# SowpatiLab/ribbit

Hardware: AMD Instinct MI355X
Metric: Gbases/s scanned (m=2..100) (higher is better)
Workload: dtype u32 bit planes

## Files before the change

ribbit_amd/csrc/kernels.hip:

```cpp
#include <hip/hip_runtime.h>

#include <algorithm>
#include <climits>
#include <type_traits>

#include "kernels.h"

namespace rb {

__device__ __forceinline__ uint32_t funnel(uint32_t hi, uint32_t lo, uint32_t sh) {
    return __builtin_amdgcn_alignbit(hi, lo, sh);
}

template <unsigned TT>
__device__ __forceinline__ uint32_t bitop3(uint32_t a, uint32_t b, uint32_t c) {
    return __builtin_amdgcn_bitop3_b32(a, b, c, TT);
}

__global__ __launch_bounds__(256) void pack_kernel(const uint8_t *__restrict__ ascii, int64_t length,
                                                   uint32_t *__restrict__ hi, uint32_t *__restrict__ lo,
                                                   uint32_t *__restrict__ brk, int64_t total_words,
                                                   uint32_t *__restrict__ zero_words, int n_zero) {
    const int64_t t = (int64_t)blockIdx.x * blockDim.x + threadIdx.x;
    if (blockIdx.x == 0)
        for (int i = threadIdx.x; i < n_zero; i += 256) zero_words[i] = 0u;
    if (t >= total_words) return;
    const int64_t p0 = (t - LEAD_WORDS) * 32;
    uint32_t h = 0, l = 0, b = 0xffffffffu;
    if (p0 >= 0 && p0 < length) {
        uint32_t w[8];
        const int64_t left = length - p0;
        const uint8_t *src = ascii + p0;
        if (left >= 32 && (((uintptr_t)src) & 15) == 0) {
            const uint4 v0 = *reinterpret_cast<const uint4 *>(src);
            const uint4 v1 = *reinterpret_cast<const uint4 *>(src + 16);
            w[0] = v0.x; w[1] = v0.y; w[2] = v0.z; w[3] = v0.w;
            w[4] = v1.x; w[5] = v1.y; w[6] = v1.z; w[7] = v1.w;
        } else {
#pragma unroll
            for (int i = 0; i < 8; i++) {
                uint32_t x = 0;
#pragma unroll
                for (int k = 0; k < 4; k++) {
                    const int idx = 4 * i + k;
                    const uint32_t c = (idx < left) ? (uint32_t)src[idx] : (uint32_t)'N';
                    x |= c << (8 * k);
                }
                w[i] = x;
            }
        }
        b = 0;
#pragma unroll
        for (int i = 0; i < 8; i++) {
            const uint32_t x = w[i];
            const uint32_t b2 = (x >> 2) & 0x01010101u;
            const uint32_t lo1 = ((x >> 1) & 0x01010101u) ^ b2;
            const uint32_t both = lo1 & b2, either = lo1 | b2;
            uint32_t expect = (either << 1) + 0x61616161u;
            expect = (b2 << 2) + expect;
            expect = (both << 3) + expect;
            expect = (both << 2) + expect;
            expect = both + expect;
            const uint32_t diff = (x | 0x20202020u) ^ expect;
            const uint32_t nz = (((diff & 0x7f7f7f7fu) + 0x7f7f7f7fu) | diff) & 0x80808080u;
            const uint32_t bad = nz >> 7;
            const uint32_t ok = bad ^ 0x01010101u;
            const uint32_t weights = 0x08040201u;
            h |= __builtin_amdgcn_udot4(b2 & ok, weights, 0u, false) << (4 * i);
            l |= __builtin_amdgcn_udot4(lo1 & ok, weights, 0u, false) << (4 * i);
            b |= __builtin_amdgcn_udot4(bad, weights, 0u, false) << (4 * i);
        }
        if (left < 32) b |= 0xffffffffu << (uint32_t)left;
    }
    hi[t] = h; lo[t] = l; brk[t] = b;
}

void launch_pack(const uint8_t *dev_ascii, int64_t length, uint32_t *hi, uint32_t *lo, uint32_t *brk,
                 int64_t total_words, uint32_t *zero_words, int n_zero, hipStream_t stream) {
    const int threads = 256;
    const int64_t blocks = (total_words + threads - 1) / threads;
    hipLaunchKernelGGL(pack_kernel, dim3((unsigned)blocks), dim3(threads), 0, stream, dev_ascii, length, hi, lo, brk,
                       total_words, zero_words, n_zero);
}

constexpr int EV_STAGE = 256;

__device__ __forceinline__ int wave_inclusive_scan(int v) {
    v += __builtin_amdgcn_update_dpp(0, v, 0x111, 0xf, 0xf, true);
    v += __builtin_amdgcn_update_dpp(0, v, 0x112, 0xf, 0xf, true);
    v += __builtin_amdgcn_update_dpp(0, v, 0x114, 0xf, 0xf, true);
    v += __builtin_amdgcn_update_dpp(0, v, 0x118, 0xf, 0xf, true);
    v += __builtin_amdgcn_update_dpp(0, v, 0x142, 0xa, 0xf, false);
    v += __builtin_amdgcn_update_dpp(0, v, 0x143, 0xc, 0xf, false);
    return v;
}

struct EventSink {
    uint64_t *events;
    uint32_t *counters;
    uint32_t region_cap;
    uint32_t shard;
};

__device__ __forceinline__ void sink_flush(const EventSink &sk, volatile uint64_t *stage, int &staged, int lane) {
    if (staged == 0) return;
    uint32_t base = 0;
    if (lane == 0) base = atomicAdd(&sk.counters[sk.shard * EV_COUNTER_STRIDE], (uint32_t)staged);
    base = (uint32_t)__builtin_amdgcn_readfirstlane((int)base);
    uint64_t *dst = sk.events + (size_t)sk.shard * sk.region_cap;
    for (int i = lane; i < staged; i += 64) {
        const uint32_t idx = base + (uint32_t)i;
        if (idx < sk.region_cap) dst[idx] = stage[i];
    }
    __builtin_amdgcn_wave_barrier();
    staged = 0;
}

template <typename EndKind>
__device__ __forceinline__ void stage_events(const uint32_t (&S)[WORDS_PER_LANE], const uint32_t (&E)[WORDS_PER_LANE],
                                             uint32_t word0, uint32_t mlen, const EventSink &sink,
                                             volatile uint64_t *stage, int &staged, int lane, EndKind end_kind) {
    uint32_t Sv[WORDS_PER_LANE], Ev[WORDS_PER_LANE];
#pragma unroll
    for (int k = 0; k < WORDS_PER_LANE; k++) {
        Sv[k] = S[k]; Ev[k] = E[k];
        asm volatile("" : "+v"(Sv[k]), "+v"(Ev[k]));
    }
    int cnt = 0;
#pragma unroll
    for (int k = 0; k < WORDS_PER_LANE; k++) cnt += __popc(Sv[k]) + __popc(Ev[k]);
    const int incl = wave_inclusive_scan(cnt);
    const int total = __builtin_amdgcn_readlane(incl, 63);
    if (staged + total > EV_STAGE) sink_flush(sink, stage, staged, lane);
    const bool direct = total > EV_STAGE;
    uint32_t idx = (uint32_t)(incl - cnt);
    uint64_t *gdst = nullptr;
    if (direct) {
        uint32_t base = 0;
        if (lane == 0) base = atomicAdd(&sink.counters[sink.shard * EV_COUNTER_STRIDE], (uint32_t)total);
        idx += (uint32_t)__builtin_amdgcn_readfirstlane((int)base);
        gdst = sink.events + (size_t)sink.shard * sink.region_cap;
    } else {
        idx += (uint32_t)staged;
    }
#pragma unroll
    for (int k = 0; k < WORDS_PER_LANE; k++) {
        uint32_t both = Sv[k] | Ev[k];
        while (both) {
            const uint32_t b = (uint32_t)__builtin_ctz(both);
            both &= both - 1u;
            const uint32_t pos = ((word0 + (uint32_t)k) << 5) + b;
            const uint32_t kind = ((Sv[k] >> b) & 1u) ? (uint32_t)EV_START : end_kind(k, b, pos);
            const uint64_t e = ev_pack(pos, mlen, kind);
            if (direct) { if (idx < sink.region_cap) gdst[idx] = e; }
            else stage[idx] = e;
            idx++;
        }
    }
    if (!direct) staged += total;
    __builtin_amdgcn_wave_barrier();
}

constexpr int K = WORDS_PER_LANE;

#ifndef RB_COOP_MAX_LANES
#define RB_COOP_MAX_LANES 16
#endif
constexpr int COOP_SRC = 16;
struct CoopScratch { uint32_t w[COOP_SRC][20]; };

__device__ __forceinline__ void stage_events_coop(const uint32_t (&S)[WORDS_PER_LANE], const uint32_t (&E)[WORDS_PER_LANE], uint32_t word0, uint32_t mlen,
                                                  uint32_t brk_at, const uint32_t *s_brk, uint32_t length, CoopScratch &sc, const EventSink &sink,
                                                  volatile uint64_t *stage, int &staged, int lane) {
    uint32_t Sv[WORDS_PER_LANE], Ev[WORDS_PER_LANE];
#pragma unroll
    for (int k = 0; k < WORDS_PER_LANE; k++) {
        Sv[k] = S[k]; Ev[k] = E[k];
        asm volatile("" : "+v"(Sv[k]), "+v"(Ev[k]));
    }
    int cnt = 0;
#pragma unroll
    for (int k = 0; k < WORDS_PER_LANE; k++) cnt += __popc(Sv[k] | Ev[k]);
    const int incl = wave_inclusive_scan(cnt);
    const int total = __builtin_amdgcn_readlane(incl, 63);
    if (staged + total > EV_STAGE) sink_flush(sink, stage, staged, lane);
    const bool direct = total > EV_STAGE;
    uint32_t first = (uint32_t)(incl - cnt);
    uint64_t *gdst = nullptr;
    if (direct) {
        uint32_t base = 0;
        if (lane == 0) base = atomicAdd(&sink.counters[sink.shard * EV_COUNTER_STRIDE], (uint32_t)total);
        first += (uint32_t)__builtin_amdgcn_readfirstlane((int)base);
        gdst = sink.events + (size_t)sink.shard * sink.region_cap;
    } else {
        first += (uint32_t)staged;
    }
    unsigned long long todo = __ballot(cnt != 0);
    const int r = lane >> 2, j = lane & 3;
    do {
        const int rank = (int)__builtin_amdgcn_mbcnt_hi((uint32_t)(todo >> 32), __builtin_amdgcn_mbcnt_lo((uint32_t)todo, 0u));
        const bool mine = ((todo >> lane) & 1ull) != 0ull && rank < COOP_SRC;
        if (mine) {
            uint32_t *row = sc.w[rank];
#pragma unroll
            for (int k = 0; k < WORDS_PER_LANE; k++) { row[k] = Sv[k]; row[WORDS_PER_LANE + k] = Ev[k]; }
            row[16] = word0; row[17] = mlen; row[18] = brk_at; row[19] = first;
        }
        const unsigned long long handled = __ballot(mine);
        const int nsrc = __popcll(handled);
        todo &= ~handled;
        __builtin_amdgcn_wave_barrier();
        uint32_t s0 = 0, s1 = 0, e0 = 0, e1 = 0;
        if (r < nsrc) { s0 = sc.w[r][2 * j]; s1 = sc.w[r][2 * j + 1]; e0 = sc.w[r][WORDS_PER_LANE + 2 * j]; e1 = sc.w[r][WORDS_PER_LANE + 2 * j + 1]; }
        const int c = __popc(s0 | e0) + __popc(s1 | e1);
        const int q0 = __builtin_amdgcn_update_dpp(0, c, 0x00, 0xf, 0xf, true);
        const int q1 = __builtin_amdgcn_update_dpp(0, c, 0x55, 0xf, 0xf, true);
        const int q2 = __builtin_amdgcn_update_dpp(0, c, 0xaa, 0xf, 0xf, true);
        if (c != 0) {
            const uint32_t w0 = sc.w[r][16], ml = sc.w[r][17], bb = sc.w[r][18];
            uint32_t idx = sc.w[r][19] + (uint32_t)((j > 0 ? q0 : 0) + (j > 1 ? q1 : 0) + (j > 2 ? q2 : 0));
            auto expand = [&](uint32_t sw, uint32_t ew, uint32_t k) {
                uint32_t both = sw | ew;
                while (both) {
                    const uint32_t b = (uint32_t)__builtin_ctz(both);
                    both &= both - 1u;
                    const uint32_t pos = ((w0 + k) << 5) + b;
                    uint32_t kind = (uint32_t)EV_START;
                    if (!((sw >> b) & 1u))
                        kind = pos >= length ? (uint32_t)EV_END_EOS : (((s_brk[bb + k] >> b) & 1u) ? (uint32_t)EV_END_N : (uint32_t)EV_END_ZERO);
                    const uint64_t e = ev_pack(pos, ml, kind);
                    if (direct) { if (idx < sink.region_cap) gdst[idx] = e; }
                    else stage[idx] = e;
                    idx++;
                }
            };
            expand(s0, e0, 2u * (uint32_t)j);
            expand(s1, e1, 2u * (uint32_t)j + 1u);
        }
        __builtin_amdgcn_wave_barrier();
    } while (RB_COOP_MAX_LANES > COOP_SRC && todo != 0ull);
    if (!direct) staged += total;
}
__device__ __forceinline__ void group_filter(const uint32_t (&PASS)[K + 2], const uint32_t (&EVAL)[K + 2], int tj, uint32_t (&SV)[K + 1],
                                             uint32_t (&DR)[K]) {
    uint32_t J[K + 2], W[K + 2];
#pragma unroll
    for (int j = K + 1; j >= 1; j--) J[j] = PASS[j] | funnel(PASS[j], PASS[j - 1], 31);
    J[0] = PASS[0] | (PASS[0] << 1);
#pragma unroll
    for (int j = K + 1; j >= 1; j--) J[j] = J[j] | funnel(J[j], J[j - 1], 30);
    J[0] = J[0] | (J[0] << 2);
#pragma unroll
    for (int j = K + 1; j >= 1; j--) J[j] = J[j] | funnel(J[j], J[j - 1], 28);
    J[0] = J[0] | (J[0] << 4);
#pragma unroll
    for (int j = 0; j < K + 1; j++) J[j] = J[j] & funnel(J[j + 1], J[j], 1);
    J[K + 1] = J[K + 1] & (J[K + 1] >> 1);
#pragma unroll
    for (int j = 0; j < K + 1; j++) J[j] = J[j] & funnel(J[j + 1], J[j], 2);
    J[K + 1] = J[K + 1] & (J[K + 1] >> 2);
#pragma unroll
    for (int j = 0; j < K + 1; j++) J[j] = J[j] & funnel(J[j + 1], J[j], 4);
    J[K + 1] = J[K + 1] & (J[K + 1] >> 4);
#pragma unroll
    for (int j = 0; j < K + 2; j++) J[j] |= PASS[j];
#pragma unroll
    for (int j = 0; j < K + 2; j++) W[j] = J[j];
    {
        int span = 1;
#pragma unroll
        for (int step = 0; step < 4; step++) {
            const int sh = min(span, tj - span);
            if (sh > 0) {
#pragma unroll
                for (int j = 0; j < K + 1; j++) W[j] = W[j] & funnel(W[j + 1], W[j], (uint32_t)sh);
                W[K + 1] = W[K + 1] & (W[K + 1] >> sh);
                span += sh;
            }
        }
        span = 1;
#pragma unroll
        for (int step = 0; step < 4; step++) {
            const int sh = min(span, tj - span);
            if (sh > 0) {
#pragma unroll
                for (int j = K + 1; j >= 1; j--) W[j] = W[j] | funnel(W[j], W[j - 1], (uint32_t)(32 - sh));
                W[0] = W[0] | (W[0] << sh);
                span += sh;
            }
        }
    }
    auto special_ends = [&](int j) {
        const uint32_t jprev = j > 0 ? funnel(J[j], J[j - 1], 31) : (J[0] << 1);
        const uint32_t ev8 = j < K + 1 ? funnel(EVAL[j + 1], EVAL[j], 8) : (EVAL[K + 1] >> 8);
        const uint32_t g = ~J[j] & jprev & ~(EVAL[j] & ev8);
        return j == 0 ? 0u : (j == K + 1 ? (g & 0x0000ffffu) : g);
    };
    uint32_t special = 0;
#pragma unroll
    for (int j = 1; j < K + 2; j++) special |= special_ends(j);
    if (__ballot(special != 0) != 0ull) {
        uint32_t G[K + 2], JL[K + 2];
#pragma unroll
        for (int j = 0; j < K + 2; j++) { JL[j] = J[j]; G[j] = special_ends(j); }
#pragma unroll
        for (int j = 0; j < K + 1; j++) G[j] = funnel(G[j + 1], G[j], 1) & J[j];
        G[K + 1] = (G[K + 1] >> 1) & J[K + 1];
#pragma unroll
        for (int sh = 1; sh <= 8; sh <<= 1) {
#pragma unroll
            for (int j = 0; j < K + 1; j++) G[j] |= funnel(G[j + 1], G[j], (uint32_t)sh) & JL[j];
            G[K + 1] |= (G[K + 1] >> sh) & JL[K + 1];
#pragma unroll
            for (int j = 0; j < K + 1; j++) JL[j] = JL[j] & funnel(JL[j + 1], JL[j], (uint32_t)sh);
            JL[K + 1] = JL[K + 1] & (JL[K + 1] >> sh);
        }
#pragma unroll
        for (int j = 0; j < K + 1; j++) W[j] |= G[j];
    }
#pragma unroll
    for (int j = 0; j < K + 1; j++) SV[j] = W[j];
#pragma unroll
    for (int k = 0; k < K; k++) {
        const uint32_t jprev = funnel(J[k + 1], J[k], 31);
        const uint32_t svprev = funnel(W[k + 1], W[k], 31);
        DR[k] = ~J[k + 1] & jprev & ~svprev;
    }
}

constexpr int LDS_EXTRA = 40;

template <bool UNIFORM>
__device__ __forceinline__ uint32_t perfect_edges(const uint32_t (&Z)[K + 2], uint32_t t3, uint32_t t4, uint32_t t5,
                                                  uint32_t back, uint32_t (&SQ)[K], uint32_t (&EQ)[K]) {
    uint32_t D[K + 2];
#pragma unroll
    for (int j = 0; j < K + 1; j++) D[j] = Z[j] | funnel(Z[j + 1], Z[j], 1);
    D[K + 1] = Z[K + 1] | (Z[K + 1] >> 1);
#pragma unroll
    for (int j = 0; j < K + 1; j++) D[j] = D[j] | funnel(D[j + 1], D[j], 2);
    D[K + 1] = D[K + 1] | (D[K + 1] >> 2);
#pragma unroll
    for (int j = 0; j < K + 1; j++) D[j] = D[j] | funnel(D[j + 1], D[j], t3);
    D[K + 1] = D[K + 1] | (D[K + 1] >> t3);
#pragma unroll
    for (int j = 0; j < K + 1; j++) D[j] = D[j] | funnel(D[j + 1], D[j], t4);
    if (!UNIFORM || t5) {
        D[K + 1] = D[K + 1] | (D[K + 1] >> t4);
#pragma unroll
        for (int j = 0; j < K + 1; j++) D[j] = D[j] | funnel(D[j + 1], D[j], t5);
    }
    uint32_t any = 0;
#pragma unroll
    for (int k = 0; k < K; k++) {
        const int j = k + 1;
        const uint32_t prev_z = funnel(Z[j], Z[j - 1], 31);
        const uint32_t d_back = funnel(D[j], D[j - 1], back);
        SQ[k] = prev_z & ~D[j];
        EQ[k] = Z[j] & ~d_back;
        any = bitop3<0xFE>(SQ[k], EQ[k], any);
    }
    return any;
}

constexpr int CAND_CAP = 64;
#ifndef RB_CAND_DIRECT
#define RB_CAND_DIRECT 32
#endif
constexpr int CAND_DIRECT = RB_CAND_DIRECT;
struct CandQueue {
    uint32_t z[K + 2][CAND_CAP];
    uint32_t tag[CAND_CAP];
};

#ifndef RB_PERFECT_WAVES
#define RB_PERFECT_WAVES 4
#endif
__global__ __launch_bounds__(256) __attribute__((amdgpu_waves_per_eu(RB_PERFECT_WAVES, RB_PERFECT_WAVES))) void scan_perfect_kernel(DevicePlanes pl, PerfectLaunch pp, int motifs_per_block,
                                                           uint64_t *__restrict__ events,
                                                           uint32_t *__restrict__ counters) {
    __shared__ uint32_t s_hi[TILE_WORDS + LDS_EXTRA];
    __shared__ uint32_t s_lo[TILE_WORDS + LDS_EXTRA];
    __shared__ uint32_t s_brk[TILE_WORDS + 8];
    __shared__ uint64_t s_stage[4][EV_STAGE];
    __shared__ CandQueue s_cand[4];
    __shared__ CoopScratch s_coop[4];

    const int lane = threadIdx.x & 63;
    const int wave = __builtin_amdgcn_readfirstlane((int)(threadIdx.x >> 6));
    const int64_t tile_base = (int64_t)blockIdx.x * TILE_WORDS;

    const int bm_lo = pp.m_lo + (int)blockIdx.y * motifs_per_block;
    const int bm_hi = min(pp.m_hi, bm_lo + motifs_per_block - 1);
    const int q_hi = bm_hi >> 5;

    const int n_ext = TILE_WORDS + 4 + q_hi;
    for (int i = threadIdx.x; i < n_ext; i += 256) {
        s_hi[i] = pl.hi[tile_base - 1 + i];
        s_lo[i] = pl.lo[tile_base - 1 + i];
    }
    for (int i = threadIdx.x; i < TILE_WORDS + 2; i += 256) s_brk[i] = pl.brk[tile_base - 1 + i];
    __syncthreads();

    const int wm_lo = bm_lo + wave;
    const int wm_hi = bm_hi;
    if (wm_lo > wm_hi) return;

    const int lb = lane * K;
    uint32_t H[K + 2], Lo[K + 2], Bk[K + 2];
#pragma unroll
    for (int j = 0; j < K + 2; j++) { H[j] = s_hi[lb + j]; Lo[j] = s_lo[lb + j]; Bk[j] = s_brk[lb + j]; }

    uint32_t Hq[K + 3], Lq[K + 3];
    int cur_q = -1;
    const uint32_t length = (uint32_t)pl.length;
    const uint32_t word0 = (uint32_t)(tile_base + lb);

    EventSink sink;
    sink.events = events;
    sink.counters = counters;
    sink.region_cap = pp.ev_cap / EV_SHARDS;
    sink.shard = (blockIdx.x * 4u + (uint32_t)wave + blockIdx.y) % EV_SHARDS;
    volatile uint64_t *stage = s_stage[wave];
    int staged = 0;

    CandQueue &cq = s_cand[wave];
    int queued = 0;
    auto flush_candidates = [&]() {
        if (queued == 0) return;
        const bool live = lane < queued;
        const uint32_t tag = live ? cq.tag[lane] : 0u;
        const uint32_t src = tag & 0xffu, qm = tag >> 8;
        uint32_t Zq[K + 2];
#pragma unroll
        for (int j = 0; j < K + 2; j++) Zq[j] = live ? cq.z[j][lane] : 0xffffffffu;
        const int c1 = (qm <= 6u) ? 12 - (int)qm : (int)qm;
        const int sp = live ? min(c1, 32) : 32;
        const uint32_t t3 = (uint32_t)min(4, sp - 4);
        const uint32_t t4 = (uint32_t)min(8, sp - 4 - (int)t3);
        const uint32_t t5 = (uint32_t)(sp - 4) - t3 - t4;
        uint32_t SQ[K], EQ[K];
        uint32_t any = perfect_edges<false>(Zq, t3, t4, t5, 32u - (uint32_t)sp, SQ, EQ);
        if (!live) {
            any = 0;
#pragma unroll
            for (int k = 0; k < K; k++) { SQ[k] = 0; EQ[k] = 0; }
        }
#ifdef RB_ABLATE_STAGING
        const unsigned long long with_events = __ballot(any == 0xdeadbeefu);
#else
        const unsigned long long with_events = __ballot(any != 0);
#endif
        if (with_events != 0ull) {
            const uint32_t src_word0 = (uint32_t)tile_base + src * (uint32_t)K;
            if (__popcll(with_events) <= RB_COOP_MAX_LANES)
                stage_events_coop(SQ, EQ, src_word0, qm, src * (uint32_t)K + 1u, s_brk, length, s_coop[wave], sink, stage, staged, lane);
            else
                stage_events(SQ, EQ, src_word0, qm, sink, stage, staged, lane, [&](int k, uint32_t b, uint32_t pos) {
                    if (pos >= length) return (uint32_t)EV_END_EOS;
                    return ((s_brk[src * (uint32_t)K + (uint32_t)k + 1u] >> b) & 1u) ? (uint32_t)EV_END_N : (uint32_t)EV_END_ZERO;
                });
        }
        queued = 0;
        __builtin_amdgcn_wave_barrier();
    };

    for (int m = wm_lo; m <= wm_hi; m += 4) {
        const int q = m >> 5;
        const uint32_t r = (uint32_t)m & 31u;
        if (q != cur_q) {
            cur_q = q;
#pragma unroll
            for (int j = 0; j < K + 3; j++) { Hq[j] = s_hi[lb + j + q]; Lq[j] = s_lo[lb + j + q]; }
        }
        const int c1 = (m <= 6) ? 12 - m : m;
        const int sp = min(c1, 32);
        const uint32_t t3 = (uint32_t)min(4, sp - 4);
        const uint32_t t4 = (uint32_t)min(8, sp - 4 - (int)t3);
        const uint32_t t5 = (uint32_t)(sp - 4) - t3 - t4;

        uint32_t Z[K + 2];
#pragma unroll
        for (int j = 0; j < K + 2; j++) {
            const uint32_t hs = funnel(Hq[j + 1], Hq[j], r);
            const uint32_t ls = funnel(Lq[j + 1], Lq[j], r);
            Z[j] = bitop3<0xF6>(bitop3<0xBE>(H[j], hs, Bk[j]), Lo[j], ls);
        }
        if (sp >= 7) {
            bool cand;
            if (sp >= 31) {
                typedef unsigned short half2 __attribute__((ext_vector_type(2)));
                auto pk_min = [](uint32_t a, uint32_t b) {
                    const half2 m = __builtin_elementwise_min(__builtin_bit_cast(half2, a), __builtin_bit_cast(half2, b));
                    return __builtin_bit_cast(uint32_t, m);
                };
                uint32_t lowest = Z[0];
#pragma unroll
                for (int j = 1; j < K + 2; j++) lowest = pk_min(lowest, Z[j]);
                cand = (((lowest - 0x00010001u) & ~lowest) & 0x80008000u) != 0;
            } else {
                const uint32_t ones = sp >= 15 ? 0x01010101u : 0x11111111u;
                const uint32_t tops = sp >= 15 ? 0x80808080u : 0x88888888u;
                uint32_t hit = 0;
#pragma unroll
                for (int j = 0; j < K + 2; j++) hit = bitop3<0xBA>(Z[j] - ones, Z[j], hit);
                cand = (hit & tops) != 0;
            }
#ifdef RB_ABLATE_CHAIN
            const unsigned long long mask = __ballot(cand && Z[0] == 0xdeadbeefu);
#else
            const unsigned long long mask = __ballot(cand);
#endif
            if (mask == 0ull) continue;
            const int n = __popcll(mask);
            if (n <= CAND_DIRECT) {
                if (queued + n > CAND_CAP) flush_candidates();
                if (cand) {
                    const int slot = queued + (int)__builtin_amdgcn_mbcnt_hi((uint32_t)(mask >> 32), __builtin_amdgcn_mbcnt_lo((uint32_t)mask, 0u));
#pragma unroll
                    for (int j = 0; j < K + 2; j++) cq.z[j][slot] = Z[j];
                    cq.tag[slot] = (uint32_t)lane | ((uint32_t)m << 8);
                }
                queued += n;
                __builtin_amdgcn_wave_barrier();
                continue;
            }
        }
        uint32_t SQ[K], EQ[K];
        const uint32_t any = perfect_edges<true>(Z, t3, t4, t5, 32u - (uint32_t)sp, SQ, EQ);
#ifdef RB_ABLATE_STAGING
        const unsigned long long with_events = __ballot(any == 0xdeadbeefu);
#else
        const unsigned long long with_events = __ballot(any != 0);
#endif
        if (with_events != 0ull) {
            if (__popcll(with_events) <= RB_COOP_MAX_LANES)
                stage_events_coop(SQ, EQ, word0, (uint32_t)m, (uint32_t)lb + 1u, s_brk, length, s_coop[wave], sink, stage, staged, lane);
            else
                stage_events(SQ, EQ, word0, (uint32_t)m, sink, stage, staged, lane, [&](int k, uint32_t b, uint32_t pos) {
                    if (pos >= length) return (uint32_t)EV_END_EOS;
                    return ((Bk[k + 1] >> b) & 1u) ? (uint32_t)EV_END_N : (uint32_t)EV_END_ZERO;
                });
        }
    }
    flush_candidates();
    sink_flush(sink, stage, staged, lane);
}

static ScanSplit scan_split(const PerfectLaunch &pp, int nm, int64_t want_y, int max_y) {
    int motifs_per_block;
    if (pp.motifs_per_block > 0) {
        motifs_per_block = std::min(pp.motifs_per_block, nm);
    } else {
        const int gy = (int)(want_y < 1 ? 1 : (want_y > max_y ? max_y : want_y));
        motifs_per_block = (nm + gy - 1) / gy;
    }
    ScanSplit sp;
    sp.motifs_per_block = motifs_per_block;
    sp.grid_y = (nm + motifs_per_block - 1) / motifs_per_block;
    return sp;
}

ScanSplit launch_scan_perfect(const DevicePlanes &pl, const PerfectLaunch &pp, uint64_t *events, uint32_t *counters,
                              hipStream_t stream) {
    const int nm = pp.m_hi - pp.m_lo + 1;
    if (nm <= 0 || pl.ntiles <= 0) return {};
    const ScanSplit sp = scan_split(pp, nm, (2048 + pl.ntiles - 1) / pl.ntiles, (nm + 3) / 4);
    dim3 grid((unsigned)pl.ntiles, (unsigned)sp.grid_y);
    hipLaunchKernelGGL(scan_perfect_kernel, grid, dim3(256), 0, stream, pl, pp, sp.motifs_per_block, events, counters);
    return sp;
}

template <int ALLOWED>
__global__ __launch_bounds__(256) void scan_window_kernel(DevicePlanes pl, PerfectLaunch pp, int motifs_per_block,
                                                          uint64_t *__restrict__ events,
                                                          uint32_t *__restrict__ counters) {
    __shared__ uint32_t s_hi[TILE_WORDS + LDS_EXTRA];
    __shared__ uint32_t s_lo[TILE_WORDS + LDS_EXTRA];
    __shared__ uint32_t s_brk[TILE_WORDS + 8];
    __shared__ uint64_t s_stage[4][EV_STAGE];

    const int lane = threadIdx.x & 63;
    const int wave = __builtin_amdgcn_readfirstlane((int)(threadIdx.x >> 6));
    const int64_t tile_base = (int64_t)blockIdx.x * TILE_WORDS;

    const int bm_lo = pp.m_lo + (int)blockIdx.y * motifs_per_block;
    const int bm_hi = min(pp.m_hi, bm_lo + motifs_per_block - 1);
    const int q_hi = bm_hi >> 5;
    const int n_ext = TILE_WORDS + 4 + q_hi;
    for (int i = threadIdx.x; i < n_ext; i += 256) {
        s_hi[i] = pl.hi[tile_base - 1 + i];
        s_lo[i] = pl.lo[tile_base - 1 + i];
    }
    for (int i = threadIdx.x; i < TILE_WORDS + 2; i += 256) s_brk[i] = pl.brk[tile_base - 1 + i];
    __syncthreads();

    const int wm_lo = bm_lo + wave;
    const int wm_hi = bm_hi;
    if (wm_lo > wm_hi) return;

    const int lb = lane * K;
    uint32_t H[K + 2], Lo[K + 2];
    uint32_t EVAL[K + 1];
    {
        uint32_t B[K + 2];
#pragma unroll
        for (int j = 0; j < K + 2; j++) { H[j] = s_hi[lb + j]; Lo[j] = s_lo[lb + j]; B[j] = s_brk[lb + j]; }
#pragma unroll
        for (int j = 0; j < K + 1; j++) B[j] |= funnel(B[j + 1], B[j], 1);
        B[K + 1] |= B[K + 1] >> 1;
#pragma unroll
        for (int j = 0; j < K + 1; j++) B[j] |= funnel(B[j + 1], B[j], 2);
        B[K + 1] |= B[K + 1] >> 2;
#pragma unroll
        for (int j = 0; j < K + 1; j++) EVAL[j] = ~(B[j] | funnel(B[j + 1], B[j], 4));
    }

    uint32_t Hq[K + 3], Lq[K + 3];
    int cur_q = -1;
    const uint32_t length = (uint32_t)pl.length;
    const uint32_t word0 = (uint32_t)(tile_base + lb);

    EventSink sink;
    sink.events = events;
    sink.counters = counters;
    sink.region_cap = pp.ev_cap / EV_SHARDS;
    sink.shard = (blockIdx.x * 4u + (uint32_t)wave + blockIdx.y) % EV_SHARDS;
    volatile uint64_t *stage = s_stage[wave];
    int staged = 0;

    for (int m = wm_lo; m <= wm_hi; m += 4) {
        const int q = m >> 5;
        const uint32_t r = (uint32_t)m & 31u;
        if (q != cur_q) {
            cur_q = q;
#pragma unroll
            for (int j = 0; j < K + 3; j++) { Hq[j] = s_hi[lb + j + q]; Lq[j] = s_lo[lb + j + q]; }
        }
        uint32_t A1[K + 2], B1[K + 2], C1[K + 2];
#pragma unroll
        for (int j = 0; j < K + 2; j++) {
            const uint32_t hs = funnel(Hq[j + 1], Hq[j], r);
            const uint32_t ls = funnel(Lq[j + 1], Lq[j], r);
            A1[j] = (H[j] ^ hs) | (Lo[j] ^ ls);
        }
#pragma unroll
        for (int j = 0; j < K + 2; j++) {
            const uint32_t sa = (j <= K) ? funnel(A1[j + 1 <= K + 1 ? j + 1 : j], A1[j], 1) : (A1[j] >> 1);
            B1[j] = A1[j] & sa;
            A1[j] = A1[j] | sa;
        }
#pragma unroll
        for (int j = 0; j < K + 2; j++) {
            const uint32_t sa = (j <= K) ? funnel(A1[j + 1 <= K + 1 ? j + 1 : j], A1[j], 2) : (A1[j] >> 2);
            const uint32_t sb = (j <= K) ? funnel(B1[j + 1 <= K + 1 ? j + 1 : j], B1[j], 2) : (B1[j] >> 2);
            if (ALLOWED == 2) C1[j] = (B1[j] & sa) | (A1[j] & sb);
            B1[j] = B1[j] | sb | (A1[j] & sa);
            A1[j] = A1[j] | sa;
        }
        uint32_t PASS[K + 1];
#pragma unroll
        for (int j = 0; j < K + 1; j++) {
            const uint32_t sa = funnel(A1[j + 1], A1[j], 4);
            const uint32_t sb = funnel(B1[j + 1], B1[j], 4);
            uint32_t bad;
            if (ALLOWED == 2) {
                const uint32_t sc = funnel(C1[j + 1], C1[j], 4);
                bad = C1[j] | sc | (B1[j] & sa) | (A1[j] & sb);
            } else {
                bad = B1[j] | sb | (A1[j] & sa);
            }
            PASS[j] = EVAL[j] & ~bad;
        }
        uint32_t ST[K], EN[K];
        uint32_t any = 0;
#pragma unroll
        for (int k = 0; k < K; k++) {
            const uint32_t prev = funnel(PASS[k + 1], PASS[k], 31);
            ST[k] = PASS[k + 1] & ~prev;
            EN[k] = ~PASS[k + 1] & prev;
            any |= ST[k] | EN[k];
        }
        if (__ballot(any != 0) != 0ull) {
            stage_events(ST, EN, word0, (uint32_t)m, sink, stage, staged, lane, [&](int k, uint32_t b, uint32_t pos) {
                if ((EVAL[k + 1] >> b) & 1u) return (uint32_t)EV_END_ZERO;
                return (pos + 7u >= length) ? (uint32_t)EV_END_EOS : (uint32_t)EV_END_N;
            });
        }
    }
    sink_flush(sink, stage, staged, lane);
}

ScanSplit launch_scan_window(const DevicePlanes &pl, const PerfectLaunch &pp, int allowed_mismatches, uint64_t *events,
                             uint32_t *counters, hipStream_t stream) {
    const int nm = pp.m_hi - pp.m_lo + 1;
    if (nm <= 0 || pl.ntiles <= 0) return {};
    const ScanSplit sp = scan_split(pp, nm, (2048 + pl.ntiles - 1) / pl.ntiles, (nm + 3) / 4);
    dim3 grid((unsigned)pl.ntiles, (unsigned)sp.grid_y);
    if (allowed_mismatches == 1)
        hipLaunchKernelGGL(scan_window_kernel<1>, grid, dim3(256), 0, stream, pl, pp, sp.motifs_per_block, events, counters);
    else
        hipLaunchKernelGGL(scan_window_kernel<2>, grid, dim3(256), 0, stream, pl, pp, sp.motifs_per_block, events, counters);
    return sp;
}

constexpr int RUN_SAT = 1 << 20;

__global__ __launch_bounds__(256) __attribute__((amdgpu_waves_per_eu(2, 4))) void scan_anchored_kernel(DevicePlanes pl, PerfectLaunch pp, int motifs_per_block, int hl,
                                                            uint32_t *__restrict__ xa, int64_t xa_stride) {
    __shared__ uint32_t s_hi[64 * K + LDS_EXTRA];
    __shared__ uint32_t s_lo[64 * K + LDS_EXTRA];

    const int lane = threadIdx.x & 63;
    const int wave = __builtin_amdgcn_readfirstlane((int)(threadIdx.x >> 6));
    const int64_t tile_base = (int64_t)blockIdx.x * anchored_tile_words(hl);
    const int64_t first = tile_base - (int64_t)hl * K - 1;

    const int bm_lo = pp.m_lo + (int)blockIdx.y * motifs_per_block;
    const int bm_hi = min(pp.m_hi, bm_lo + motifs_per_block - 1);
    const int q_hi = (bm_hi + 2) >> 5;
    const int n_ext = 64 * K + 4 + q_hi;
    for (int i = threadIdx.x; i < n_ext; i += 256) {
        s_hi[i] = pl.hi[first + i];
        s_lo[i] = pl.lo[first + i];
    }
    __syncthreads();

    const int nmb = bm_hi - bm_lo + 1;
    const int per = (nmb + 3) >> 2;
    const int wm_lo = bm_lo + wave * per;
    const int wm_hi = min(bm_hi, wm_lo + per - 1);
    if (wm_lo > wm_hi) return;

    const int lb = lane * K;
    const bool own_lane = lane >= hl && lane < 64 - hl;
    uint32_t H[K + 2], Lo[K + 2];
#pragma unroll
    for (int j = 0; j < K + 2; j++) { H[j] = s_hi[lb + j]; Lo[j] = s_lo[lb + j]; }

    const int64_t w_own0 = tile_base + (int64_t)(lane - hl) * K;
    const int64_t length = pl.length;
    const int64_t lane_lo = (w_own0 - 1) * 32, lane_hi = (w_own0 + K + 1) * 32;
    const bool edge_lane = lane_lo < 0 || lane_hi > length - (int64_t)(wm_hi + 2);
    const bool edge_wave = __ballot(edge_lane) != 0ull;

    uint32_t Hq[K + 3], Lq[K + 3];
    int cur_q = -1;

    uint32_t AN[5][K + 2];
#pragma unroll
    for (int a = 0; a < 5; a++)
#pragma unroll
        for (int j = 0; j < K + 2; j++) AN[a][j] = 0;

    const int s_first = max(1, wm_lo - 2);
    const int s_last = wm_hi + 2;
    auto step = [&](auto slot_c, int s) {
        constexpr int R = decltype(slot_c)::value;
        constexpr int R1 = (R + 4) % 5, R3 = (R + 2) % 5, R4 = (R + 1) % 5;
        const int q = s >> 5;
        const uint32_t r = (uint32_t)s & 31u;
        if (q != cur_q) {
            cur_q = q;
#pragma unroll
            for (int j = 0; j < K + 3; j++) { Hq[j] = s_hi[lb + j + q]; Lq[j] = s_lo[lb + j + q]; }
        }
        uint32_t X[K];
#pragma unroll
        for (int k = 0; k < K; k++) {
            const uint32_t hs = funnel(Hq[k + 2], Hq[k + 1], r);
            const uint32_t ls = funnel(Lq[k + 2], Lq[k + 1], r);
            X[k] = ~((H[k + 1] ^ hs) | (Lo[k + 1] ^ ls));
        }
        if (edge_wave) {
#pragma unroll
            for (int k = 0; k < K; k++) {
                const int64_t bp = (w_own0 + k) * 32;
                const int64_t f = (length - s) - bp;
                const uint32_t force = f <= 0 ? 0xffffffffu : (f >= 32 ? 0u : (0xffffffffu << (uint32_t)f));
                X[k] = (bp < 0) ? 0u : (X[k] | force);
            }
        }
        const int two_s = 2 * s;
        int lead1[K], trail1[K];
        int span_lead = 0, span_trail = 0;
        bool alive = true;
#pragma unroll
        for (int k = 0; k < K; k++) {
            const uint32_t nx = ~X[k];
            lead1[k] = nx ? __builtin_ctz(nx) : 32;
            trail1[k] = nx ? __builtin_clz(nx) : 32;
            span_lead += alive ? lead1[k] : 0;
            alive = alive && (nx == 0u);
        }
        const bool span_full = alive;
        alive = true;
#pragma unroll
        for (int k = K - 1; k >= 0; k--) {
            span_trail += alive ? trail1[k] : 0;
            alive = alive && (X[k] == 0xffffffffu);
        }
        int accL = span_trail, accR = span_lead, fullL = span_full ? 1 : 0, fullR = fullL;
        for (int d = 1; d < hl; d <<= 1) {
            int a2 = __shfl_up(accL, d), f2 = __shfl_up(fullL, d);
            if (lane < d) { a2 = 0; f2 = 0; }
            accL = min(accL + (fullL ? a2 : 0), RUN_SAT);
            fullL &= f2;
            a2 = __shfl_down(accR, d); f2 = __shfl_down(fullR, d);
            if (lane + d > 63) { a2 = 0; f2 = 0; }
            accR = min(accR + (fullR ? a2 : 0), RUN_SAT);
            fullR &= f2;
        }
        int left_in = __shfl_up(accL, 1);
        int right_in = __shfl_down(accR, 1);
        if (lane == 0) left_in = 0;
        if (lane == 63) right_in = 0;
        int CL[K], CR[K];
        {
            int c = left_in;
#pragma unroll
            for (int k = 0; k < K; k++) { CL[k] = c; c = (X[k] == 0xffffffffu) ? min(c + 32, RUN_SAT) : trail1[k]; }
            c = right_in;
#pragma unroll
            for (int k = K - 1; k >= 0; k--) { CR[k] = c; c = (X[k] == 0xffffffffu) ? min(c + 32, RUN_SAT) : lead1[k]; }
        }
#pragma unroll
        for (int k = 0; k < K; k++) {
            const uint32_t x = X[k];
            const bool isfull = x == 0xffffffffu;
            const uint32_t mask_low = isfull ? 0xffffffffu : ((1u << lead1[k]) - 1u);
            const uint32_t mask_high = (isfull || trail1[k] == 0) ? 0u : (0xffffffffu << (32 - trail1[k]));
            const int low_len = CL[k] + lead1[k] + (isfull ? CR[k] : 0);
            const int high_len = trail1[k] + CR[k];
            const uint32_t inter = x & ~mask_low & ~mask_high;
            const uint32_t r3 = inter & (inter >> 1) & (inter >> 2);
            uint32_t keep = r3 | (r3 << 1) | (r3 << 2);
            if (two_s <= 30) {
                uint32_t rr = inter;
                for (int span = 1; span < two_s;) { const int sh = min(span, two_s - span); rr &= rr >> sh; span += sh; }
                for (int span = 1; span < two_s;) { const int sh = min(span, two_s - span); rr |= rr << sh; span += sh; }
                keep &= ~rr;
            }
            if (lead1[k] > 0 && low_len >= 3 && low_len < two_s) keep |= mask_low;
            if (high_len >= 3 && high_len < two_s) keep |= mask_high;
            AN[R][k + 1] = keep;
        }
// ... 639 lines not shown
```

Measured before the change: 434.3.

## Pad LDS tiles and reload per-lane words to raise waves per EU

Pads the shared hi/lo/brk tiles with one extra word every eight to spread strided per-lane LDS accesses across banks. Raises the waves-per-EU target from 4 to 5 and, to fit the smaller register budget, rematerializes the per-lane H/Lo/Bk/Hq/Lq words from LDS after each motif instead of keeping them live, and reads break bits from LDS in the event lambdas. On candidate-queue overflow it flushes, reloads and retries the motif. The gain depends on whether the extra occupancy outweighs the added LDS traffic and address arithmetic.

```diff
diff --git a/ribbit_amd/csrc/kernels.hip b/ribbit_amd/csrc/kernels.hip
--- a/ribbit_amd/csrc/kernels.hip
+++ b/ribbit_amd/csrc/kernels.hip
@@ -167,6 +167,12 @@
 #define RB_COOP_MAX_LANES 16
 #endif
 constexpr int COOP_SRC = 16;
+
+#ifndef RB_TILE_PAD
+#define RB_TILE_PAD 1
+#endif
+__host__ __device__ constexpr uint32_t tile_at(uint32_t i) { return RB_TILE_PAD ? i + (i >> 3) : i; }
+
 struct CoopScratch { uint32_t w[COOP_SRC][20]; };
 
 __device__ __forceinline__ void stage_events_coop(const uint32_t (&S)[WORDS_PER_LANE], const uint32_t (&E)[WORDS_PER_LANE], uint32_t word0, uint32_t mlen,
@@ -227,7 +233,7 @@
                     const uint32_t pos = ((w0 + k) << 5) + b;
                     uint32_t kind = (uint32_t)EV_START;
                     if (!((sw >> b) & 1u))
-                        kind = pos >= length ? (uint32_t)EV_END_EOS : (((s_brk[bb + k] >> b) & 1u) ? (uint32_t)EV_END_N : (uint32_t)EV_END_ZERO);
+                        kind = pos >= length ? (uint32_t)EV_END_EOS : (((s_brk[tile_at(bb + k)] >> b) & 1u) ? (uint32_t)EV_END_N : (uint32_t)EV_END_ZERO);
                     const uint64_t e = ev_pack(pos, ml, kind);
                     if (direct) { if (idx < sink.region_cap) gdst[idx] = e; }
                     else stage[idx] = e;
@@ -374,14 +380,14 @@
 };
 
 #ifndef RB_PERFECT_WAVES
-#define RB_PERFECT_WAVES 4
+#define RB_PERFECT_WAVES 5
 #endif
 __global__ __launch_bounds__(256) __attribute__((amdgpu_waves_per_eu(RB_PERFECT_WAVES, RB_PERFECT_WAVES))) void scan_perfect_kernel(DevicePlanes pl, PerfectLaunch pp, int motifs_per_block,
                                                            uint64_t *__restrict__ events,
                                                            uint32_t *__restrict__ counters) {
-    __shared__ uint32_t s_hi[TILE_WORDS + LDS_EXTRA];
-    __shared__ uint32_t s_lo[TILE_WORDS + LDS_EXTRA];
-    __shared__ uint32_t s_brk[TILE_WORDS + 8];
+    __shared__ uint32_t s_hi[tile_at(TILE_WORDS + LDS_EXTRA)];
+    __shared__ uint32_t s_lo[tile_at(TILE_WORDS + LDS_EXTRA)];
+    __shared__ uint32_t s_brk[tile_at(TILE_WORDS + 8)];
     __shared__ uint64_t s_stage[4][EV_STAGE];
     __shared__ CandQueue s_cand[4];
     __shared__ CoopScratch s_coop[4];
@@ -396,10 +402,10 @@
 
     const int n_ext = TILE_WORDS + 4 + q_hi;
     for (int i = threadIdx.x; i < n_ext; i += 256) {
-        s_hi[i] = pl.hi[tile_base - 1 + i];
-        s_lo[i] = pl.lo[tile_base - 1 + i];
-    }
-    for (int i = threadIdx.x; i < TILE_WORDS + 2; i += 256) s_brk[i] = pl.brk[tile_base - 1 + i];
+        s_hi[tile_at(i)] = pl.hi[tile_base - 1 + i];
+        s_lo[tile_at(i)] = pl.lo[tile_base - 1 + i];
+    }
+    for (int i = threadIdx.x; i < TILE_WORDS + 2; i += 256) s_brk[tile_at(i)] = pl.brk[tile_base - 1 + i];
     __syncthreads();
 
     const int wm_lo = bm_lo + wave;
@@ -408,11 +414,18 @@
 
     const int lb = lane * K;
     uint32_t H[K + 2], Lo[K + 2], Bk[K + 2];
-#pragma unroll
-    for (int j = 0; j < K + 2; j++) { H[j] = s_hi[lb + j]; Lo[j] = s_lo[lb + j]; Bk[j] = s_brk[lb + j]; }
-
     uint32_t Hq[K + 3], Lq[K + 3];
-    int cur_q = -1;
+    int cur_q;
+    auto load_tile = [&](int q) {
+        uint32_t at = tile_at((uint32_t)lb);
+        asm volatile("" : "+v"(at));
+#pragma unroll
+        for (int j = 0; j < K + 2; j++) { H[j] = s_hi[at + tile_at(j)]; Lo[j] = s_lo[at + tile_at(j)]; Bk[j] = s_brk[at + tile_at(j)]; }
+#pragma unroll
+        for (int j = 0; j < K + 3; j++) { Hq[j] = s_hi[at + tile_at((uint32_t)(j + q))]; Lq[j] = s_lo[at + tile_at((uint32_t)(j + q))]; }
+        cur_q = q;
+    };
+    load_tile(wm_lo >> 5);
     const uint32_t length = (uint32_t)pl.length;
     const uint32_t word0 = (uint32_t)(tile_base + lb);
 
@@ -458,7 +471,7 @@
             else
                 stage_events(SQ, EQ, src_word0, qm, sink, stage, staged, lane, [&](int k, uint32_t b, uint32_t pos) {
                     if (pos >= length) return (uint32_t)EV_END_EOS;
-                    return ((s_brk[src * (uint32_t)K + (uint32_t)k + 1u] >> b) & 1u) ? (uint32_t)EV_END_N : (uint32_t)EV_END_ZERO;
+                    return ((s_brk[tile_at(src * (uint32_t)K + (uint32_t)k + 1u)] >> b) & 1u) ? (uint32_t)EV_END_N : (uint32_t)EV_END_ZERO;
                 });
         }
         queued = 0;
@@ -471,7 +484,10 @@
         if (q != cur_q) {
             cur_q = q;
 #pragma unroll
-            for (int j = 0; j < K + 3; j++) { Hq[j] = s_hi[lb + j + q]; Lq[j] = s_lo[lb + j + q]; }
+            for (int j = 0; j < K + 3; j++) {
+                Hq[j] = s_hi[tile_at((uint32_t)lb) + tile_at((uint32_t)(j + q))];
+                Lq[j] = s_lo[tile_at((uint32_t)lb) + tile_at((uint32_t)(j + q))];
+            }
         }
         const int c1 = (m <= 6) ? 12 - m : m;
         const int sp = min(c1, 32);
@@ -514,7 +530,12 @@
             if (mask == 0ull) continue;
             const int n = __popcll(mask);
             if (n <= CAND_DIRECT) {
-                if (queued + n > CAND_CAP) flush_candidates();
+                if (queued + n > CAND_CAP) {
+                    flush_candidates();
+                    load_tile(q);
+                    m -= 4;
+                    continue;
+                }
                 if (cand) {
                     const int slot = queued + (int)__builtin_amdgcn_mbcnt_hi((uint32_t)(mask >> 32), __builtin_amdgcn_mbcnt_lo((uint32_t)mask, 0u));
 #pragma unroll
@@ -539,9 +560,10 @@
             else
                 stage_events(SQ, EQ, word0, (uint32_t)m, sink, stage, staged, lane, [&](int k, uint32_t b, uint32_t pos) {
                     if (pos >= length) return (uint32_t)EV_END_EOS;
-                    return ((Bk[k + 1] >> b) & 1u) ? (uint32_t)EV_END_N : (uint32_t)EV_END_ZERO;
+                    return ((s_brk[tile_at((uint32_t)(lb + k + 1))] >> b) & 1u) ? (uint32_t)EV_END_N : (uint32_t)EV_END_ZERO;
                 });
         }
+        load_tile(min(m + 4, wm_hi) >> 5);
     }
     flush_candidates();
     sink_flush(sink, stage, staged, lane);
```

After: 434.0, median of 2. No clear change (-0.1%).
